# melspectrum007/audio-visual-speech-enhancement

Measured on AMD Instinct MI355X. Metric: clips/sec (STFT+CNN forward) on 200-ms@16kHz segments, 1/2/4/8 MI355X, higher is better.
Workload: dtype fp32_split

## Files before the change

audio-visual-speech-enhancement_amd/csrc/avse_common.h:

```cpp
#pragma once
#include <hip/hip_runtime.h>
#include <stdint.h>
#include <string>

typedef __bf16 bf16_t;
typedef __bf16 bf16x8 __attribute__((ext_vector_type(8)));
typedef _Float16 f16x8 __attribute__((ext_vector_type(8)));
typedef _Float16 f16x4 __attribute__((ext_vector_type(4)));
typedef float f32x4 __attribute__((ext_vector_type(4)));
typedef int i32x4 __attribute__((ext_vector_type(4)));

struct avse_ctx;

namespace avse {

void set_error(const std::string& msg);

int ctx_device_index(const struct ::avse_ctx* c);

int ensure_lds_attr(const void* fn, int bytes);

struct Options {
    int no_gemm = 0;
    int no_audenc = 0;
    int no_dechead = 0;
    int no_dectail = 0;
    int unfused_tail = 0;
    int no_halo = 0;
    int mfma32 = 0;
    int serial = 0;
    int graph = 0;
    int gemm_ksplit_cap = 0;
    int dense_istft = 0;
    int no_act_scale = 0;
    int no_win = 0;
    int no_v1p = 0;
    int no_a1valu = 0;
    int side_prio = 0;
};

#define AVSE_HIP_CHECK(expr)                                                                   \
    do {                                                                                       \
        hipError_t _e = (expr);                                                                \
        if (_e != hipSuccess) {                                                                \
            ::avse::set_error(std::string(#expr " failed: ") + hipGetErrorString(_e));         \
            return 2;                                                        \
        }                                                                                      \
    } while (0)

struct DebugHit {
    unsigned hit, kernel, code, block, thread;
    int value, expect;
};
enum DebugKernel : unsigned {
    DK_V1R = 1,
    DK_SPEC = 3,
    DK_ISTFT = 4,
};
#ifdef AVSE_DEBUG
inline constexpr bool kDebugBuild = true;
__device__ __forceinline__ void debug_record(DebugHit* h, unsigned kern, unsigned code, int value, int expect) {
    if (atomicCAS(&h->hit, 0u, 1u) == 0u) {
        h->kernel = kern;
        h->code = code;
        h->block = blockIdx.x;
        h->thread = threadIdx.x;
        h->value = value;
        h->expect = expect;
        __threadfence();
    }
}
#define AVSE_DEBUG_RECORD(reader)                                                                    \
    static __device__ ::avse::DebugHit g_avse_dbg;                                                   \
    int reader(::avse::DebugHit* out) {                                                              \
        ::avse::DebugHit zero{};                                                                     \
        if (hipMemcpyFromSymbol(out, HIP_SYMBOL(g_avse_dbg), sizeof(zero)) != hipSuccess) return 2;   \
        return hipMemcpyToSymbol(HIP_SYMBOL(g_avse_dbg), &zero, sizeof(zero)) == hipSuccess ? 0 : 2; \
    }
#define AVSE_CHECK_DEV(cond, kern, code, value, expect)                                              \
    do {                                                                                             \
        if (!(cond)) ::avse::debug_record(&g_avse_dbg, (kern), (code), (int)(value), (int)(expect)); \
    } while (0)
#else
inline constexpr bool kDebugBuild = false;
#define AVSE_DEBUG_RECORD(reader)              \
    int reader(::avse::DebugHit* out) {          \
        *out = ::avse::DebugHit{};               \
        return 0;                                \
    }
#define AVSE_CHECK_DEV(cond, kern, code, value, expect) \
// ... 168 lines not shown
    const bf16_t* w1;
    const bf16_t* w2;
    const bf16_t* w3;
    const float* sc[3];
    const float* sh[3];
};
bool dec_head_supported(const DecHeadArgs& a);
int launch_dec_head(const DecHeadArgs& a, hipStream_t s);

struct GemmArgs {
    const bf16_t* a;
    long long lda;
    const bf16_t* w;
    int M, N, kpad;
    const float* scale;
    const float* shift;
    int act;
    bf16_t* out;
    long long ldo;
    int out_off;
    int ksplit;
    float* partial;
    int* counters;
    int split;
    int slabs_per_split;
    unsigned* range_flag;
    unsigned range_bit;
};
int gemm_ksplit(int M, int N, int kpad, int cap);
int gemm_s16_ksplit(int N, int kpad, int* slabs_per_split);
size_t gemm_ws_bytes(int M, int N, int kpad, int cap);
int launch_gemm(const GemmArgs& g, int mode, hipStream_t s);
int launch_aud_enc(const AudEncArgs& a, hipStream_t s);
int launch_dec_tail(const DecTailArgs& a, hipStream_t s);

enum HaloVariant { HALO_NONE = -1, HALO_V1 = 0, HALO_K5 = 1, HALO_K3_16 = 2, HALO_K3_8 = 3, HALO_V1P = 4 };
enum HaloOut { OUT_BF16 = 0, OUT_S16 = 1, OUT_F32 = 2 };

struct HaloArgs {
    int variant;
    const void* in;
    const float* video;
    const float* vmean;
    const float* vstd;
    void* out;
    const void* w;
    const float* scale;
    const float* shift;
    int N, Hc, Wc, Ci, Co;
    long long out_clip_stride;
    int out_pix_stride;
    int out_c_off;
    int mfma32;
    int split;
    int out_mode;
    unsigned long long* prof;
    unsigned* range_flag;
    unsigned range_bit, range_in_bit;
};

int launch_conv_stream(const HaloArgs& a, hipStream_t s);
int launch_conv_v1r(const HaloArgs& a, hipStream_t s);
int launch_video_prep(const float* video, const float* mean, const float* stdv, void* out, int64_t N,
                      int F, int dtype, hipStream_t s);
int launch_audio_prep(const float* audio, void* out, int64_t npix, int dtype, hipStream_t s);
int launch_aconv1_split(const float* in, const float* w, const float* scale, const float* shift, void* out, int64_t N,
                        int H, int W, int Ho, int Wo, int KH, int KW, int S, int pt, int pl, int Co, unsigned* range_flag,
                        unsigned range_bit, unsigned range_in_bit, hipStream_t s);
int launch_out_conv(const void* in, const float* w64, float bias, float* out, int64_t npix, int dtype,
                    hipStream_t s);
int launch_broadcast_row(const void* src, void* dst, int64_t rows, int64_t row_bytes, int64_t stride_bytes,
                         hipStream_t s);
int launch_video_normalize(float* video, int64_t S, int H, int W, int F, const float* mean,
                           const float* stdv, hipStream_t s);
int launch_mse(const float* a, const float* b, int64_t n, float* loss, float* partial, hipStream_t s);

size_t mix_pairs_scratch_bytes(int64_t n_pairs);
int launch_mix_pairs(const int16_t* speech, const int64_t* speech_off, const int16_t* noise, const int64_t* noise_off,
                     const double* snr_lin, int64_t n_pairs, int64_t L, float* rows, double* mix64, double* factor,
                     void* scratch, hipStream_t s);
constexpr int kVideoStatsMaxF = 8;
size_t video_stats_scratch_bytes(int64_t S, int H, int W);
int launch_video_stats(const float* video, int64_t S, int H, int W, int F, float* mean, float* stdv, void* scratch,
                       hipStream_t s);

}
```

audio-visual-speech-enhancement_amd/csrc/capi.hip:

```cpp
#include <algorithm>
#include <atomic>
#include <cmath>
#include <cstdio>
#include <cstdlib>
#include <cstring>
#include <mutex>
#include <set>
#include <string>
#include <utility>
#include <vector>

#include "../../include/avse.h"
#include "avse_common.h"
#include "netplan.h"

namespace avse {
static thread_local std::string g_err;
void set_error(const std::string& msg) { g_err = msg; }

int ensure_lds_attr(const void* fn, int bytes) {
    static std::mutex mu;
    static std::set<std::pair<const void*, int>> done;
    int dev = 0;
    AVSE_HIP_CHECK(hipGetDevice(&dev));
// ... 112 lines not shown
    struct Graph {
        const void* key[9];
        int64_t n;
        Options opt;
        hipGraphExec_t exec;
    };
    std::vector<Graph> graphs;
    hipStream_t cap = nullptr;
};

namespace avse {
int ctx_device_index(const avse_ctx* c) { return c->device; }
}

struct GpuLayer {
    LayerDef def;
    int cin_pad = 0;
    int hq = 0, wq = 0, ho = 0, wo = 0;
    int nphase = 1;
    ConvPhase ph[MAX_PHASES];
    void* w = nullptr;
    float* scale = nullptr;
    float* shift = nullptr;
    int2* taps = nullptr;
    int halo = HALO_NONE;
    void* w_halo = nullptr;
    void* w_dense = nullptr;
    float* w_f32 = nullptr;
    float* scale_h = nullptr;
    int2 htaps[MAX_TAPS * MAX_PHASES] = {};
};

struct OptionName {
    const char* name;
    const char* env;
    int Options::*field;
};
const OptionName kOptionNames[] = {
    {"no_gemm", "AVSE_NO_GEMM", &Options::no_gemm},
    {"no_audenc", "AVSE_NO_AUDENC", &Options::no_audenc},
    {"no_dechead", "AVSE_NO_DECHEAD", &Options::no_dechead},
    {"no_dectail", "AVSE_NO_DECTAIL", &Options::no_dectail},
    {"unfused_tail", "AVSE_UNFUSED_TAIL", &Options::unfused_tail},
    {"no_halo", "AVSE_NO_HALO", &Options::no_halo},
    {"mfma32", "AVSE_MFMA32", &Options::mfma32},
    {"serial", "AVSE_SERIAL", &Options::serial},
    {"graph", "AVSE_GRAPH", &Options::graph},
    {"gemm_ksplit_cap", "AVSE_GEMM_KSPLIT", &Options::gemm_ksplit_cap},
    {"dense_istft", "AVSE_DENSE_ISTFT", &Options::dense_istft},
    {"no_act_scale", "AVSE_NO_ACT_SCALE", &Options::no_act_scale},
    {"no_win", "AVSE_NO_WIN", &Options::no_win},
    {"no_v1p", "AVSE_NO_V1P", &Options::no_v1p},
    {"no_a1valu", "AVSE_NO_A1VALU", &Options::no_a1valu},
    {"side_prio", "AVSE_SIDE_PRIO", &Options::side_prio},
};

struct avse_weights {
    int dtype = 0;
    int device = 0;
    uint64_t serial = 0;
    NetPlan plan = kPlan25;
    GpuLayer layers[kNumLayers - 1];
    float* d6_w = nullptr;
    float d6_bias = 0.f;
    mutable std::atomic<void*> vzero_emb{nullptr};
    mutable std::mutex vzero_mu;
    mutable unsigned vzero_range = 0;
    int act_exp[kNumLayers] = {};
    std::vector<float> blob;
    mutable avse_weights* f32_twin = nullptr;
    mutable std::mutex twin_mu;
    std::vector<void*> allocs;
    ~avse_weights();
};

avse_weights::~avse_weights() {
    delete f32_twin;
    (void)hipFree(vzero_emb.load());
    for (void* p : allocs) (void)hipFree(p);
}

namespace {

template <typename T>
int upload(avse_weights* W, const std::vector<T>& h, T** out) {
    void* p = nullptr;
    if (hipMalloc(&p, sizeof(T) * (h.empty() ? 1 : h.size())) != hipSuccess) return fail(AVSE_ERR_OOM, "hipMalloc failed (weights)");
    W->allocs.push_back(p);
    if (!h.empty() && hipMemcpy(p, h.data(), sizeof(T) * h.size(), hipMemcpyHostToDevice) != hipSuccess)
        return fail(AVSE_ERR_HIP, "hipMemcpy failed (weights)");
    *out = (T*)p;
    return 0;
}

struct Arena {
    size_t off[32];
    size_t per_clip_bytes;
};
enum Buf { B_VIN, B_AIN, B_A1, B_A2, B_A3, B_A4, B_V1, B_V2, B_V3, B_V4, B_V5, B_CAT, B_E1, B_E2, B_E3,
           B_D1, B_D2, B_D3, B_D4, B_D5, B_COUNT };
size_t buf_elems(const NetPlan& p, int b) {
    const size_t T = p.T, w1 = (T + 1) / 2, w3 = p.W5;
    const size_t e[B_COUNT] = {128 * 128 * 8, 80 * T * 8, 40 * w1 * 64, 40 * w1 * 64, 20 * w3 * 128,
                               10 * w3 * 128, 64 * 64 * 128, 32 * 32 * 128, 16 * 16 * 256, 8 * 8 * 256,
                               4 * 4 * 512, (size_t)p.cat, (size_t)p.emb, (size_t)p.emb, (size_t)p.aemb,
                               10 * w3 * 128, 20 * w3 * 128, 40 * 2 * w3 * 128, 40 * 2 * w3 * 64, 80 * 4 * w3 * 64};
// ... 532 lines not shown
                            const uint16_t h = f2h(v);
                            sp[((size_t)st * L.cout + n) * 32 + kk] = h;
                            sp[((size_t)st * L.cout + n) * 32 + 16 + kk] = f2h(v - h2f(h));
                        }
            }
            if ((rc = upload(W, scale_h, &G.scale_h))) return rc;
            uint16_t* d;
            if ((rc = upload(W, sp, &d))) return rc;
            G.w_halo = d;
            return 0;
        }
        if ((rc = upload(W, scale_h, &G.scale_h))) return rc;
        std::vector<uint16_t> hp;
        if (G.halo == HALO_V1) {
            hp.assign((size_t)L.kh * L.cout * 32, 0);
            for (int ky = 0; ky < L.kh; ++ky)
                for (int n = 0; n < L.cout; ++n)
                    for (int kx = 0; kx < L.kw; ++kx)
                        for (int f = 0; f < L.cin; ++f)
                            hp[((size_t)ky * L.cout + n) * 32 + kx * 6 + f] =
                                f2bf(sgn[n] * kernel[((size_t)(ky * L.kw + kx) * L.cin + f) * L.cout + n]);
        } else {
            const int nsteps = (L.cin / 128) * 4 * ntap;
            hp.assign((size_t)nsteps * L.cout * 32, 0);
            for (int st = 0; st < nsteps; ++st)
                for (int n = 0; n < L.cout; ++n)
                    for (int kk = 0; kk < 32; ++kk) {
                        const int tap = st % ntap, chunk = st / ntap;
                        const int c = chunk * 32 + kk;
                        hp[((size_t)st * L.cout + n) * 32 + kk] =
                            f2bf(sgn[n] * kernel[((size_t)tap * L.cin + c) * L.cout + n]);
                    }
        }
        uint16_t* d;
        if ((rc = upload(W, hp, &d))) return rc;
        G.w_halo = d;
    }
    return 0;
}

HaloArgs halo_args(const GpuLayer& G, const void* in, const float* video, const float* vmean, const float* vstd,
                   void* out, long long out_clip_stride, int out_pix_stride, int out_c_off, int64_t N,
                   const Options& opt) {
    HaloArgs a;
    std::memset(&a, 0, sizeof(a));
    a.variant = G.halo;
    a.in = in;
    a.video = video;
    a.vmean = vmean;
    a.vstd = vstd;
    a.out = out;
    a.w = G.w_halo;
    a.mfma32 = opt.mfma32;
    a.scale = G.scale_h;
    a.shift = G.shift;
    a.N = (int)N;
    a.Hc = G.def.hin;
    a.Wc = G.def.win;
    a.Ci = G.def.cin;
    a.Co = G.def.cout;
    a.out_clip_stride = out_clip_stride;
    a.out_pix_stride = out_pix_stride;
    a.out_c_off = out_c_off;
    return a;
}

DecTailArgs dec_tail_args(const GpuLayer& G4, const GpuLayer& G5, const avse_weights* W, const void* in, float* out,
                          int64_t N) {
    DecTailArgs a;
    std::memset(&a, 0, sizeof(a));
    a.in = reinterpret_cast<const bf16_t*>(in);
    a.out = out;
    a.N = (int)N;
    auto extents = [](const GpuLayer& G, int p, int& dy0, int& dy1, int& dx0, int& dx1) {
        dy0 = dx0 = 1 << 20;
        dy1 = dx1 = -(1 << 20);
        for (int t = 0; t < G.ph[p].ntaps; ++t) {
            const int2 d = G.htaps[G.ph[p].tap_off + t];
            dy0 = std::min(dy0, d.x); dy1 = std::max(dy1, d.x);
            dx0 = std::min(dx0, d.y); dx1 = std::max(dx1, d.y);
        }
    };
    a.w4 = reinterpret_cast<const bf16_t*>(G4.w);
    a.sc4 = G4.scale;
    a.sh4 = G4.shift;
    a.nt4 = G4.ph[0].ntaps;
    a.kpad4 = G4.ph[0].kpad;
    int dy0, dy1, dx0, dx1;
    extents(G4, 0, dy0, dy1, dx0, dx1);
    a.pt4 = -dy0; a.pl4 = -dx0; a.rows4 = G4.hq + dy1 - dy0; a.pitch4 = G4.wq + dx1 - dx0;
    bool grid_ok = true;
    auto tap_grid = [&](const GpuLayer& G, int p, int& dy, int& dx, int& nx) {
        const int2* t = G.htaps + G.ph[p].tap_off;
        const int nt = G.ph[p].ntaps;
        dy = t[0].x;
        dx = t[0].y;
        nx = 1;
        while (nx < nt && t[nx].x == dy) ++nx;
        for (int k = 0; k < nt; ++k)
            if (t[k].x != dy - k / nx || t[k].y != dx - k % nx) grid_ok = false;
    };
    tap_grid(G4, 0, a.dy4, a.dx4, a.nx4);
    a.w5 = reinterpret_cast<const bf16_t*>(G5.w);
    a.sc5 = G5.scale;
    a.sh5 = G5.shift;
    int ey0 = 1 << 20, ey1 = -(1 << 20), ex0 = 1 << 20, ex1 = -(1 << 20);
// ... 899 lines not shown
```

audio-visual-speech-enhancement_amd/csrc/conv_stream.hip:

```cpp
#include <cstdlib>
#include <type_traits>

#include "avse_common.h"

namespace avse {
namespace {

constexpr float LRELU = 0.3f;
constexpr int kOOB = 0x7fffff00;

typedef float f32x16 __attribute__((ext_vector_type(16)));

template <bool M16> __device__ __forceinline__ int wswz(int row) { return M16 ? 2 * ((row >> 2) & 1) : (row >> 2) & 3; }
template <bool M16> __device__ __forceinline__ int hsw(int y) { return M16 ? 2 * (y & 1) : y & 3; }

__device__ __forceinline__ __amdgpu_buffer_rsrc_t make_rsrc(const void* base, long long bytes) {
    const int nrec = bytes > kOOB ? kOOB : (bytes < 0 ? 0 : (int)bytes);
    return __builtin_amdgcn_make_buffer_rsrc(const_cast<void*>(base), (short)0, nrec, 0x00020000);
}

#ifndef AVSE_HALO_AUX
#define AVSE_HALO_AUX 0
#endif
#ifndef AVSE_WGT_AUX
#define AVSE_WGT_AUX 0
#endif
__device__ __forceinline__ i32x4 ld16(__amdgpu_buffer_rsrc_t rs, int voff, int soff) {
    return __builtin_amdgcn_raw_buffer_load_b128(rs, voff, soff, AVSE_HALO_AUX);
}
__device__ __forceinline__ i32x4 ld16w(__amdgpu_buffer_rsrc_t rs, int voff, int soff) {
    return __builtin_amdgcn_raw_buffer_load_b128(rs, voff, soff, AVSE_WGT_AUX);
}
__device__ __forceinline__ void st16(char* p, i32x4 v) { *reinterpret_cast<i32x4*>(p) = v; }

template <int N>
__device__ __forceinline__ void wait_vm_lgkm0() {
    static_assert(N >= 0 && N < 64, "vmcnt range");
    asm volatile("s_waitcnt vmcnt(%0) lgkmcnt(0)" ::"n"(N) : "memory");
}
__device__ __forceinline__ void barrier_raw() { asm volatile("s_barrier" ::: "memory"); }

template <int KS, int TH, int TW, int NCLIP, int LAT_ = (KS == 5 ? 10 : 6), int BP_ = 1, bool S16_ = false>
struct StreamGeom {
    static constexpr int HH = TH + KS - 1, HW = TW + KS - 1;
    static constexpr int HPIX = NCLIP * HH * HW;
    static constexpr int HPIECES = (HPIX * 64 + 1023) / 1024;
    static constexpr int HPW = (HPIECES + 3) / 4;
    static constexpr int NTAP = KS * KS;
    static constexpr int CSLOT = HPIECES * 1024;
    static constexpr int WSLOT = 8192;
    static constexpr int LAT = LAT_, BP = BP_, NWS = S16_ ? 2 * BP + 1 : 2 * BP, WD = LAT + BP + 1, NHS = 3,
                         PAIR = ((2 * NTAP) % BP ? 4 : 2) * NTAP, CPI = PAIR / NTAP;
    static_assert(PAIR % BP == 0, "barrier periods align with the unrolled loader iteration");
    static_assert(BP == 1 || BP == 2 || (S16_ && BP == 4), "barrier period");
    static_assert(!S16_ || BP % 2 == 0, "split-f16 operands: whole slice pairs per barrier");
    static constexpr int LDS = NHS * CSLOT + NWS * WSLOT;
    static_assert(LDS + 1024 <= 160 * 1024, "LDS");
    static_assert(NCLIP * TH * TW == 256, "tile = 256 conv pixels (4 waves x 4 fragments)");
    static_assert(PAIR % LAT == 0 && LAT < NTAP, "the ring set of a step is compile-time");
    static_assert(HPW <= NTAP && HPW - 1 + LAT + BP - 1 <= 2 * NTAP - (S16_ ? BP + 1 : 2), "halo pieces must land in time");
    static constexpr int loads(int j, int abl) {
        const int tap = ((j % NTAP) + NTAP) % NTAP;
        return ((abl & 2) ? 0 : 2) + ((!(abl & 1) && tap < HPW) ? 1 : 0);
    }
    static constexpr int vm_wait(int j, int abl) {
        int n = 0;
        for (int i = j - LAT + 2; i <= j; ++i) n += loads(i, abl);
        return n;
    }
};

template <int KS, int TH, int TW, int NCLIP, bool M16 = true, int LAT_ = StreamGeom<KS, TH, TW, NCLIP>::LAT, int ABL = 0,
          int BP_ = 1, bool S16 = false>
__global__ __launch_bounds__(512, 1) void k_conv_stream(HaloArgs a) {
    static_assert(!S16 || M16, "split-f16 operands: 16x16x32 compute waves only");
    using G = StreamGeom<KS, TH, TW, NCLIP, LAT_, BP_, S16>;
    constexpr int HH = G::HH, HW = G::HW, HPIX = G::HPIX, HPW = G::HPW, NTAP = G::NTAP;
    constexpr int CSLOT = G::CSLOT, WSLOT = G::WSLOT, LAT = G::LAT, WD = G::WD, PAIR = G::PAIR;
    constexpr int BP = G::BP, NWS = G::NWS;
    constexpr int BPR = TW / 8, BPC = (TH / 4) * BPR;
    static_assert(TW % 8 == 0 && TH % 4 == 0 && BPC % 2 == 0, "a wave's two blocks share their y origin mod 4");
    constexpr int PAD = (KS - 1) / 2;

    extern __shared__ __attribute__((aligned(1024))) char lds[];
    char* const halo = lds;
    char* const wring = lds + G::NHS * CSLOT;

    const int tid = threadIdx.x;
    const int lane = tid & 63;
    const int wave = __builtin_amdgcn_readfirstlane(tid >> 6);
    const int w = wave & 3;

    const int nch = a.Ci / 32;
    const int spt = nch * NTAP;
    const int tiles_x = a.Wc / TW, tiles_y = a.Hc / TH;
    const int tiles_per_clip = tiles_x * tiles_y;
    const int ntiles = ((a.N + NCLIP - 1) / NCLIP) * tiles_per_clip;
    const int gxs = (int)gridDim.x;
    const int slot = (gxs % 8 == 0) ? ((int)blockIdx.x % 8) * (gxs / 8) + (int)blockIdx.x / 8 : (int)blockIdx.x;
    const int nmine = (ntiles - slot + gxs - 1) / gxs;
    if (nmine <= 0) return;
    const int nchunks = nmine * nch;
    const int co0 = blockIdx.y * 128;
    const long long clip_bytes = (long long)a.Hc * a.Wc * a.Ci * 2;

    auto tile_origin = [&](int k, int& clip0, int& oy0, int& ox0) {
        const int t = slot + k * gxs;
        clip0 = (ABL & 64) ? 0 : (t / tiles_per_clip) * NCLIP;
        const int tt = t % tiles_per_clip;
        oy0 = (tt / tiles_x) * TH;
        ox0 = (tt % tiles_x) * TW;
    };

    if (wave >= 4) {
        const __amdgpu_buffer_rsrc_t wrs = make_rsrc(reinterpret_cast<const char*>(a.w) + (size_t)co0 * 64,
                                                     (long long)spt * a.Co * 64 - (long long)co0 * 64);
        const int wslice = a.Co * 64, wend = spt * wslice;
        int wvoff[2];
#pragma unroll
        for (int u = 0; u < 2; ++u) {
            const int row = 32 * w + 16 * u + (lane >> 2), sl = lane & 3;
            wvoff[u] = row * 64 + ((sl ^ wswz<M16>(row)) << 4);
        }
        char* const wdst = wring + 2048 * w + lane * 16;
        auto tile_rsrc = [&](int clip0) {
            return make_rsrc(reinterpret_cast<const char*>(a.in) + (long long)clip0 * clip_bytes,
                             (long long)(a.N - clip0) * clip_bytes);
        };
        const int ci2 = a.Ci * 2, hc = a.Hc, wc = a.Wc;
        auto tile_voffs = [&](int oy0, int ox0, int (&vo)[HPW]) {
#pragma unroll
            for (int pc = 0; pc < HPW; ++pc) {
                const int P = w + 4 * pc;
                const int p = P * 16 + (lane >> 2), sl = lane & 3;
                const int cl = p / (HH * HW), rr = p - cl * (HH * HW);
                const int y = rr / HW, x = rr - y * HW;
                const int iy = oy0 + y - PAD, ix = ox0 + x - PAD;
                const int off = ((cl * hc + iy) * wc + ix) * ci2 + ((sl ^ hsw<M16>(y)) << 4);
                const bool ok = (P < G::HPIECES) & (p < HPIX) & ((unsigned)iy < (unsigned)hc) & ((unsigned)ix < (unsigned)wc);
                vo[pc] = ok ? off : kOOB;
            }
        };
        auto piece_store = [&](auto pcc, char* base, i32x4 v) {
            constexpr int pc = decltype(pcc)::value;
            if constexpr (4 * pc + 3 < G::HPIECES) st16(base + pc * 4096, v);
            else if (w + 4 * pc < G::HPIECES) st16(base + pc * 4096, v);
        };

        int cur_clip0, cur_oy0, cur_ox0, nxt_clip0, nxt_oy0, nxt_ox0;
        tile_origin(0, cur_clip0, cur_oy0, cur_ox0);
        tile_origin(1, nxt_clip0, nxt_oy0, nxt_ox0);
        __amdgpu_buffer_rsrc_t cur_rs = tile_rsrc(cur_clip0), nxt_rs = tile_rsrc(nxt_clip0);
        int vo_cur[HPW], vo_nxt[HPW];
        tile_voffs(cur_oy0, cur_ox0, vo_cur);
        tile_voffs(nxt_oy0, nxt_ox0, vo_nxt);
        char* const pbase0 = halo + w * 1024 + lane * 16;

        [&]<int... PC>(std::integer_sequence<int, PC...>) {
            (piece_store(std::integral_constant<int, PC>{}, pbase0, ld16(cur_rs, vo_cur[PC], 0)), ...);
            ((PC < NTAP - LAT ? piece_store(std::integral_constant<int, PC>{}, pbase0 + CSLOT, ld16(cur_rs, vo_cur[PC], 64))
                              : (void)0), ...);
        }(std::make_integer_sequence<int, HPW>{});
#pragma unroll
        for (int s = 0; s <= BP; ++s)
#pragma unroll
            for (int u = 0; u < 2; ++u) st16(wdst + s * WSLOT + 1024 * u, ld16w(wrs, wvoff[u], (s % spt) * wslice));
        i32x4 rw[LAT][2], rp[LAT];
        [&]<int... S>(std::integer_sequence<int, S...>) {
            ([&] {
                 rw[S][0] = ld16w(wrs, wvoff[0], ((S + BP + 1) % spt) * wslice);
                 rw[S][1] = ld16w(wrs, wvoff[1], ((S + BP + 1) % spt) * wslice);
                 constexpr int vt = NTAP - LAT + S;
                 if constexpr (vt < HPW && !(ABL & 1)) rp[S] = ld16(cur_rs, vo_cur[vt < HPW ? vt : 0], 64);
             }(), ...);
        }(std::make_integer_sequence<int, LAT>{});
        wait_vm_lgkm0<0>();
        barrier_raw();
        barrier_raw();

        int k = 0, c = 0, g = 0, hs2 = 2;
        int woff = (WD % spt) * wslice;
        constexpr bool kRot = PAIR % NWS != 0;
        int wrot = 0;
        int vsel[HPW];
        __amdgpu_buffer_rsrc_t prs = cur_rs;
        int psoff = 0;
        char* pd_cur = pbase0 + CSLOT;
        char* pd_prev = pd_cur;
        unsigned long long ptp = (ABL & 128) ? __builtin_amdgcn_s_memtime() : 0, pt0 = 0, pt1 = 0, p_work = 0,
                           p_wait = 0, p_bar = 0;
        auto chunk_begin = [&]() {
            const bool nx = c + 2 >= nch;
            const bool real = g + 2 < nchunks;
#pragma unroll
            for (int pc = 0; pc < HPW; ++pc) vsel[pc] = !real ? kOOB : nx ? vo_nxt[pc] : vo_cur[pc];
            prs = nx ? nxt_rs : cur_rs;
            psoff = (nx ? c + 2 - nch : c + 2) * 64;
            pd_prev = pd_cur;
            pd_cur = pbase0 + hs2 * CSLOT;
        };
        auto chunk_end = [&]() {
            ++g;
            hs2 = hs2 == 2 ? 0 : hs2 + 1;
            if (++c == nch) {
                c = 0;
                ++k;
                cur_oy0 = nxt_oy0;
                cur_ox0 = nxt_ox0;
                cur_rs = nxt_rs;
#pragma unroll
                for (int pc = 0; pc < HPW; ++pc) vo_cur[pc] = vo_nxt[pc];
                tile_origin(k + 1, nxt_clip0, nxt_oy0, nxt_ox0);
                nxt_rs = tile_rsrc(nxt_clip0);
                tile_voffs(nxt_oy0, nxt_ox0, vo_nxt);
            }
        };
        auto lstep = [&](auto jidx) {
            constexpr int j = decltype(jidx)::value;
            constexpr int tap = j % NTAP, S = j % LAT;
            constexpr int jl = j - LAT;
            constexpr int tl = ((jl % NTAP) + NTAP) % NTAP;
            constexpr bool lprev = (jl < 0) || (jl / NTAP != j / NTAP);
            if constexpr (tap == 0) chunk_begin();
            if constexpr (!(ABL & 2)) {
                int wsl = (j + BP + 1) % NWS + (kRot ? wrot : 0);
                if (wsl >= NWS) wsl -= NWS;
                char* const wd = wdst + wsl * WSLOT;
                st16(wd, rw[S][0]);
                st16(wd + 1024, rw[S][1]);
            }
            if constexpr (tl < HPW && !(ABL & 1))
                piece_store(std::integral_constant<int, (tl < HPW ? tl : 0)>{}, lprev ? pd_prev : pd_cur, rp[S]);
            if constexpr (!(ABL & 2)) {
                rw[S][0] = ld16w(wrs, wvoff[0], woff);
                rw[S][1] = ld16w(wrs, wvoff[1], woff);
            }
            if constexpr (tap < HPW && !(ABL & 1)) rp[S] = ld16(prs, vsel[tap < HPW ? tap : 0], psoff);
            woff += wslice;
            if (woff == wend) woff = 0;
            if constexpr (!(ABL & 4) && j % BP == BP - 1) {
                if constexpr ((ABL & 128) != 0) pt0 = __builtin_amdgcn_s_memtime();
                wait_vm_lgkm0<G::vm_wait(j, ABL)>();
                if constexpr ((ABL & 128) != 0) pt1 = __builtin_amdgcn_s_memtime();
                barrier_raw();
                if constexpr ((ABL & 128) != 0) {
                    const unsigned long long pt2 = __builtin_amdgcn_s_memtime();
                    p_work += pt0 - ptp;
                    p_wait += pt1 - pt0;
                    p_bar += pt2 - pt1;
                    ptp = pt2;
                }
            }
            if constexpr (tap == NTAP - 1) chunk_end();
        };
        for (int pr = 0; pr < nchunks; pr += G::CPI) {
            [&]<int... J>(std::integer_sequence<int, J...>) {
                (lstep(std::integral_constant<int, J>{}), ...);
            }(std::make_integer_sequence<int, PAIR>{});
            if constexpr (kRot) wrot = (wrot + PAIR) % NWS;
        }
        wait_vm_lgkm0<0>();
        if constexpr ((ABL & 128) != 0)
            if (lane == 0) {
                unsigned long long* pr = a.prof + ((size_t)blockIdx.x * 8 + wave) * 4;
                pr[0] = p_work; pr[1] = p_wait; pr[2] = p_bar; pr[3] = (unsigned long long)nchunks * NTAP;
            }
        return;
    }

    __builtin_amdgcn_s_setprio(2);
    if constexpr (M16) {
        constexpr int SBX = TW / 4, SB = (TH / 4) * SBX;
        static_assert(TH % 4 == 0 && TW % 4 == 0 && (SBX % 4 == 0 || SBX == 2) && SB % 4 == 0, "block geometry");
        const int r16 = lane & 15, kg = lane >> 4;
        const int q = r16 >> 2, dy = (r16 >> 1) & 1, dx = r16 & 1;
        const int b0 = 4 * w, cl0 = b0 / SB, bb0 = b0 % SB;
        const int by0 = bb0 / SBX, bx0 = bb0 % SBX;
        const int ab = ((cl0 * HH + 4 * by0 + 2 * (q >> 1) + dy) * HW + 4 * bx0 + 2 * (q & 1) + dx) * 64;
// ... 30 lines not shown
#pragma unroll
        for (int i = 0; i < 4; ++i)
#pragma unroll
            for (int j = 0; j < 8; ++j) acc[i][j] = (f32x4){};
        const int Wp = a.Wc / 2;
        bool range_bad = false;
        auto epilogue_m = [&](auto modec, int clip0, int oy0, int ox0) {
            constexpr int OM = decltype(modec)::value;
            constexpr int ES = OM == OUT_F32 ? 4 : 2;
            const long long cbytes = a.out_clip_stride * ES;
            const __amdgpu_buffer_rsrc_t ors = make_rsrc(reinterpret_cast<const char*>(a.out) + (long long)clip0 * cbytes,
                                                         (long long)(a.N - clip0) * cbytes);
            const int cbase = cl0 * (int)a.out_clip_stride + a.out_c_off + (OM == OUT_S16 ? 2 * co0 : co0) + r16;
#pragma unroll
            for (int i = 0; i < 4; ++i) {
                const int py = (oy0 + 4 * (by0 + i / SBX)) / 2 + (kg >> 1);
                const int px = (ox0 + 4 * (bx0 + i % SBX)) / 2 + (kg & 1);
                const int pbase = cbase + (py * Wp + px) * a.out_pix_stride;
#pragma unroll
                for (int j = 0; j < 8; ++j) {
                    const float mx = fmaxf(fmaxf(acc[i][j][0], acc[i][j][1]), fmaxf(acc[i][j][2], acc[i][j][3]));
                    float x = fmaf(mx, ssh[16 * j + r16], ssh[128 + 16 * j + r16]);
                    x = fmaxf(x, LRELU * x);
                    if constexpr (OM == OUT_BF16) {
                        __builtin_amdgcn_raw_buffer_store_b16(__builtin_bit_cast(unsigned short, (bf16_t)x), ors,
                                                              (pbase + 16 * j) * 2, 0, 0);
                    } else if constexpr (OM == OUT_S16) {
                        const _Float16 h = (_Float16)x;
                        const _Float16 l = (_Float16)(x - (float)h);
                        range_bad |= pair_out_of_range(x);
                        __builtin_amdgcn_raw_buffer_store_b16(__builtin_bit_cast(unsigned short, h), ors,
                                                              (pbase + 32 * j) * 2, 0, 0);
                        __builtin_amdgcn_raw_buffer_store_b16(__builtin_bit_cast(unsigned short, l), ors,
                                                              (pbase + 32 * j + 16) * 2, 0, 0);
                    } else {
                        __builtin_amdgcn_raw_buffer_store_b32(__builtin_bit_cast(int, x), ors, (pbase + 16 * j) * 4, 0, 0);
                    }
                    acc[i][j] *= 0.f;
                }
            }
        };
        auto epilogue = [&](int clip0, int oy0, int ox0) {
            if constexpr (!S16) {
                epilogue_m(std::integral_constant<int, OUT_BF16>{}, clip0, oy0, ox0);
            } else if (a.out_mode == OUT_S16) {
                epilogue_m(std::integral_constant<int, OUT_S16>{}, clip0, oy0, ox0);
            } else {
                epilogue_m(std::integral_constant<int, OUT_F32>{}, clip0, oy0, ox0);
            }
        };

        unsigned long long ptp = (ABL & 128) ? __builtin_amdgcn_s_memtime() : 0, pt0 = 0, pt1 = 0, p_work = 0,
                           p_wait = 0, p_bar = 0;
        int tap1 = 1, hs1 = 0;
        i32x4 fa[4], fb[8], na[4], nb[8];
        frags(0, 0, 0, fa, fb);
        if constexpr ((ABL & 8) != 0) frags(0, 0, 0, na, nb);
        asm volatile("s_waitcnt lgkmcnt(0)" ::: "memory");
        barrier_raw();

        auto cstep = [&](auto bar, int t, i32x4 (&ca)[4], i32x4 (&cb)[8], i32x4 (&xa)[4], i32x4 (&xb)[8]) {
            if constexpr (!S16) {
                if constexpr (!(ABL & 8)) frags(hs1, tap1, (t + 1) & (NWS - 1), xa, xb);
                if constexpr (!(ABL & 16))
#pragma unroll
                    for (int i = 0; i < 4; ++i)
#pragma unroll
                        for (int j = 0; j < 8; ++j)
                            acc[i][j] = __builtin_amdgcn_mfma_f32_16x16x32_bf16(
                                __builtin_bit_cast(bf16x8, ca[i]), __builtin_bit_cast(bf16x8, cb[j]), acc[i][j], 0, 0, 0);
            }
            if constexpr (!S16) {
#pragma unroll
                for (int r = 0; r < 12; ++r) {
                    __builtin_amdgcn_sched_group_barrier(0x008, 1, 0);
                    __builtin_amdgcn_sched_group_barrier(0x100, 1, 0);
                }
                __builtin_amdgcn_sched_group_barrier(0x008, 20, 0);
                __builtin_amdgcn_sched_barrier(0);
            }
            if constexpr (!(ABL & 4) && decltype(bar)::value) {
                if constexpr ((ABL & 128) != 0) pt0 = __builtin_amdgcn_s_memtime();
                asm volatile("s_waitcnt lgkmcnt(0)" ::: "memory");
                if constexpr ((ABL & 128) != 0) pt1 = __builtin_amdgcn_s_memtime();
                barrier_raw();
                if constexpr ((ABL & 128) != 0) {
                    const unsigned long long pt2 = __builtin_amdgcn_s_memtime();
                    p_work += pt0 - ptp;
                    p_wait += pt1 - pt0;
                    p_bar += pt2 - pt1;
                    ptp = pt2;
                }
            }
            if (++tap1 == NTAP) {
                tap1 = 0;
                hs1 = hs1 == 2 ? 0 : hs1 + 1;
            }
        };
        int t = 0;
        int cur_clip0, cur_oy0, cur_ox0;
        if constexpr (S16) {
            auto advance = [&]() {
                if (++tap1 == NTAP) {
                    tap1 = 0;
                    hs1 = hs1 == 2 ? 0 : hs1 + 1;
                }
            };
            auto mfma_group = [&](const i32x4 (&ca)[4], const i32x4 (&cb)[8]) {
                if constexpr (!(ABL & 16))
#pragma unroll
                    for (int j = 0; j < 8; ++j)
#pragma unroll
                        for (int i = 0; i < 4; ++i)
                            acc[i][j] = __builtin_amdgcn_mfma_f32_16x16x32_f16(
                                __builtin_bit_cast(f16x8, ca[i]), __builtin_bit_cast(f16x8, cb[j]), acc[i][j], 0, 0, 0);
            };
            auto sched = [](auto nds, auto per) {
                constexpr int ND = decltype(nds)::value, PER = decltype(per)::value;
#pragma unroll
                for (int r = 0; r < ND; ++r) {
                    __builtin_amdgcn_sched_group_barrier(0x008, PER, 0);
                    __builtin_amdgcn_sched_group_barrier(0x100, 1, 0);
                }
                __builtin_amdgcn_sched_group_barrier(0x008, 32 - ND * PER, 0);
                __builtin_amdgcn_sched_barrier(0);
            };
            const bool hi_half = kg >= 2;
            auto pstep = [&](auto bar, int t, i32x4 (&a0)[4], i32x4 (&b0)[8], i32x4 (&na)[4], i32x4 (&nb)[8]) {
                i32x4 a1[4], b1[8], bp[8];
                const int ws0 = t % NWS, ws1 = (t + 1) % NWS, ws2 = (t + 2) % NWS;
                if constexpr (!(ABL & 8)) frags(hs1, tap1, ws1, a1, b1);
                advance();
                mfma_group(a0, b0);
                sched(std::integral_constant<int, 12>{}, std::integral_constant<int, 1>{});
                if constexpr (!(ABL & 8)) frags_lo(hi_half ? ws1 : ws0, bp);
                mfma_group(a1, b1);
                sched(std::integral_constant<int, 8>{}, std::integral_constant<int, 2>{});
#pragma unroll
                for (int i = 0; i < 4; ++i)
#pragma unroll
                    for (int d = 0; d < 4; ++d)
                        a0[i][d] = (int)__builtin_amdgcn_permlane32_swap((unsigned)a0[i][d], (unsigned)a1[i][d], false,
                                                                         false)[0];
                if constexpr (!(ABL & 8)) frags(hs1, tap1, ws2, na, nb);
                advance();
                mfma_group(a0, bp);
                sched(std::integral_constant<int, 12>{}, std::integral_constant<int, 1>{});
                if constexpr (!(ABL & 4) && decltype(bar)::value) {
                    if constexpr ((ABL & 128) != 0) pt0 = __builtin_amdgcn_s_memtime();
                    asm volatile("s_waitcnt lgkmcnt(0)" ::: "memory");
                    if constexpr ((ABL & 128) != 0) pt1 = __builtin_amdgcn_s_memtime();
                    barrier_raw();
                    if constexpr ((ABL & 128) != 0) {
                        const unsigned long long pt2 = __builtin_amdgcn_s_memtime();
                        p_work += pt0 - ptp;
                        p_wait += pt1 - pt0;
                        p_bar += pt2 - pt1;
                        ptp = pt2;
                    }
                }
            };
            for (int kt = 0; kt < nmine; ++kt) {
                for (int s = 0; s < spt; s += 4, t += 4) {
                    pstep(std::bool_constant<BP == 2>{}, t, fa, fb, na, nb);
                    pstep(std::true_type{}, t + 2, na, nb, fa, fb);
                }
                tile_origin(kt, cur_clip0, cur_oy0, cur_ox0);
                epilogue(cur_clip0, cur_oy0, cur_ox0);
            }
        } else {
            for (int kt = 0; kt < nmine; ++kt) {
                for (int s = 0; s < spt; s += 2, t += 2) {
                    cstep(std::bool_constant<BP == 1>{}, t, fa, fb, na, nb);
                    cstep(std::true_type{}, t + 1, na, nb, fa, fb);
                }
                tile_origin(kt, cur_clip0, cur_oy0, cur_ox0);
                epilogue(cur_clip0, cur_oy0, cur_ox0);
            }
        }
        if constexpr ((ABL & 128) != 0)
            if (lane == 0) {
                unsigned long long* pr = a.prof + ((size_t)blockIdx.x * 8 + wave) * 4;
                pr[0] = p_work; pr[1] = p_wait; pr[2] = p_bar; pr[3] = (unsigned long long)t;
            }
        if constexpr (S16) range_report(a.range_flag, a.range_bit, range_bad);
        return;
    }
    const int r32 = lane & 31, hi = lane >> 5;
    int ab;
    {
        const int b = 2 * w;
        const int cl = b / BPC, bb = b % BPC;
        const int q = r32 >> 2;
        const int y = 4 * (bb / BPR) + 2 * (q >> 2) + ((r32 >> 1) & 1);
        const int x = 8 * (bb % BPR) + 2 * (q & 3) + (r32 & 1);
        ab = ((cl * HH + y) * HW + x) * 64;
    }
    constexpr int blk1 = ((4 * (1 / BPR)) * HW + 8 * (1 % BPR)) * 64;
    const int ylo = 2 * ((r32 >> 4) & 1) + ((r32 >> 1) & 1);
    int boffm[2];
#pragma unroll
    for (int m = 0; m < 2; ++m) boffm[m] = r32 * 64 + (((2 * m + hi) ^ wswz<M16>(r32)) << 4);
    auto frags = [&](int hs, int tap, int ws, i32x4 (&fa)[4], i32x4 (&fb)[8]) {
        const int ky = tap / KS, kx = tap % KS;
        const int sw = hsw<M16>(ylo + ky);
        const char* hp = halo + hs * CSLOT + ab + (ky * HW + kx) * 64;
        const char* wp = wring + ws * WSLOT;
#pragma unroll
        for (int m = 0; m < 2; ++m) {
            const int pos = ((2 * m + hi) ^ sw) << 4;
#pragma unroll
            for (int i = 0; i < 2; ++i) fa[2 * i + m] = *reinterpret_cast<const i32x4*>(hp + i * blk1 + pos);
#pragma unroll
            for (int jb = 0; jb < 4; ++jb) fb[2 * jb + m] = *reinterpret_cast<const i32x4*>(wp + boffm[m] + 2048 * jb);
        }
    };
    float sc[4], sh[4];
#pragma unroll
// ... 59 lines not shown
            __builtin_amdgcn_sched_group_barrier(0x008, 1, 0);
            __builtin_amdgcn_sched_group_barrier(0x100, 1, 0);
        }
        __builtin_amdgcn_sched_group_barrier(0x008, 4, 0);
        __builtin_amdgcn_sched_barrier(0);
        if constexpr (!(ABL & 4) && decltype(bar)::value) {
            if constexpr ((ABL & 128) != 0) pt0 = __builtin_amdgcn_s_memtime();
            asm volatile("s_waitcnt lgkmcnt(0)" ::: "memory");
            if constexpr ((ABL & 128) != 0) pt1 = __builtin_amdgcn_s_memtime();
            barrier_raw();
            if constexpr ((ABL & 128) != 0) {
                const unsigned long long pt2 = __builtin_amdgcn_s_memtime();
                p_work += pt0 - ptp;
                p_wait += pt1 - pt0;
                p_bar += pt2 - pt1;
                ptp = pt2;
            }
        }
        if (++tap1 == NTAP) {
            tap1 = 0;
            hs1 = hs1 == 2 ? 0 : hs1 + 1;
        }
    };
    int t = 0;
    int cur_clip0, cur_oy0, cur_ox0;
    using BAR0 = std::bool_constant<BP == 1>;
    for (int kt = 0; kt < nmine; ++kt) {
        cstep(std::true_type{}, BAR0{}, t, fa, fb, na, nb);
        cstep(std::false_type{}, std::true_type{}, t + 1, na, nb, fa, fb);
        t += 2;
        for (int s = 2; s < spt; s += 2, t += 2) {
            cstep(std::false_type{}, BAR0{}, t, fa, fb, na, nb);
            cstep(std::false_type{}, std::true_type{}, t + 1, na, nb, fa, fb);
        }
        tile_origin(kt, cur_clip0, cur_oy0, cur_ox0);
        epilogue(cur_clip0, cur_oy0, cur_ox0);
    }
    if constexpr ((ABL & 128) != 0)
        if (lane == 0) {
            unsigned long long* pr = a.prof + ((size_t)blockIdx.x * 8 + wave) * 4;
            pr[0] = p_work; pr[1] = p_wait; pr[2] = p_bar; pr[3] = (unsigned long long)t;
        }
}

#ifndef AVSE_S16_BP5
#define AVSE_S16_BP5 4
#endif
#ifndef AVSE_S16_BP3
#define AVSE_S16_BP3 4
#endif
#ifndef AVSE_S16_LAT3
#define AVSE_S16_LAT3 4
#endif
template <int KS, int TH, int TW, int NCLIP, bool M16, bool S16 = false>
int launch_stream(const HaloArgs& a, hipStream_t s) {
    constexpr int BP = S16 ? (KS == 5 ? AVSE_S16_BP5 : AVSE_S16_BP3) : 1;
    constexpr int LAT = (S16 && KS == 3) ? AVSE_S16_LAT3 : StreamGeom<KS, TH, TW, NCLIP>::LAT;
    using G = StreamGeom<KS, TH, TW, NCLIP, LAT, BP, S16>;
    constexpr auto kern = k_conv_stream<KS, TH, TW, NCLIP, M16, G::LAT, 0, BP, S16>;
    if (int rc = ensure_lds_attr((const void*)kern, G::LDS + 1024)) return rc;
    if (a.Hc % TH || a.Wc % TW || a.Co % 128 || a.Ci % 64) {
        set_error("stream conv: tile does not divide the layer");
        return 3;
    }
    int dev = 0, ncu = 256;
    (void)hipGetDevice(&dev);
    (void)hipDeviceGetAttribute(&ncu, hipDeviceAttributeMultiprocessorCount, dev);
    const int tiles = ((a.N + NCLIP - 1) / NCLIP) * (a.Hc / TH) * (a.Wc / TW);
    const int cob = a.Co / 128;
    int gx = ncu / cob;
    gx = gx >= 8 ? gx / 8 * 8 : (gx < 1 ? 1 : gx);
    if (gx > tiles) gx = tiles;
    if ((a.Ci / 32) % G::CPI || (S16 && ((a.out_mode != OUT_S16 && a.out_mode != OUT_F32) || (a.Ci / 32 * KS * KS) % 4))) {
        set_error("stream conv: split-f16 operands write split or f32 outputs, over slice counts divisible by 4");
        return 3;
    }
    hipLaunchKernelGGL(kern, dim3(gx, cob), dim3(512), G::LDS + 1024, s, a);
    AVSE_HIP_CHECK(hipGetLastError());
    return 0;
}

}

int launch_conv_stream(const HaloArgs& a, hipStream_t s) {
    const bool m32 = a.mfma32 != 0;
    if (a.split) {
        switch (a.variant) {
            case HALO_K5: return launch_stream<5, 16, 16, 1, true, true>(a, s);
            case HALO_K3_16: return launch_stream<3, 16, 16, 1, true, true>(a, s);
            case HALO_K3_8: return launch_stream<3, 8, 8, 4, true, true>(a, s);
        }
        set_error("stream conv: unsupported variant");
        return 3;
    }
    switch (a.variant) {
        case HALO_K5: return m32 ? launch_stream<5, 16, 16, 1, false>(a, s) : launch_stream<5, 16, 16, 1, true>(a, s);
        case HALO_K3_16: return m32 ? launch_stream<3, 16, 16, 1, false>(a, s) : launch_stream<3, 16, 16, 1, true>(a, s);
        case HALO_K3_8: return m32 ? launch_stream<3, 8, 8, 4, false>(a, s) : launch_stream<3, 8, 8, 4, true>(a, s);
    }
    set_error("stream conv: unsupported variant");
    return 3;
}

}
```

Baseline: 79330.

## Add planar slice-pair pipeline for split-f16 streaming conv kernels

Adds a planar variant of the split-f16 streaming convolution main loop. It computes LDS fragment offsets incrementally with XOR-based half selection and interleaves the hi/lo fragment reads with the MFMA groups, instead of recomputing frags per step. The weight ring gains one extra look-ahead slot, with a new compile-time check that halo pieces land in time. The variant is on by default for split layers and can be disabled with AVSE_NO_PLANAR. It aims to cut address arithmetic and LDS read latency in the inner loop, at the cost of more LDS ring slots and more complex scheduling.

Result: faster. 81160, median of 6 (+2.3%).

```diff
diff --git a/audio-visual-speech-enhancement_amd/csrc/avse_common.h b/audio-visual-speech-enhancement_amd/csrc/avse_common.h
--- a/audio-visual-speech-enhancement_amd/csrc/avse_common.h
+++ b/audio-visual-speech-enhancement_amd/csrc/avse_common.h
@@ -36,6 +36,7 @@
     int no_win = 0;
     int no_v1p = 0;
     int no_a1valu = 0;
+    int no_planar = 0;
     int side_prio = 0;
 };
 
@@ -310,6 +311,7 @@
     int out_pix_stride;
     int out_c_off;
     int mfma32;
+    int no_planar;
     int split;
     int out_mode;
     unsigned long long* prof;
diff --git a/audio-visual-speech-enhancement_amd/csrc/capi.hip b/audio-visual-speech-enhancement_amd/csrc/capi.hip
--- a/audio-visual-speech-enhancement_amd/csrc/capi.hip
+++ b/audio-visual-speech-enhancement_amd/csrc/capi.hip
@@ -188,6 +188,7 @@
     {"no_win", "AVSE_NO_WIN", &Options::no_win},
     {"no_v1p", "AVSE_NO_V1P", &Options::no_v1p},
     {"no_a1valu", "AVSE_NO_A1VALU", &Options::no_a1valu},
+    {"no_planar", "AVSE_NO_PLANAR", &Options::no_planar},
     {"side_prio", "AVSE_SIDE_PRIO", &Options::side_prio},
 };
 
@@ -826,6 +827,7 @@
     a.out = out;
     a.w = G.w_halo;
     a.mfma32 = opt.mfma32;
+    a.no_planar = opt.no_planar;
     a.scale = G.scale_h;
     a.shift = G.shift;
     a.N = (int)N;
diff --git a/audio-visual-speech-enhancement_amd/csrc/conv_stream.hip b/audio-visual-speech-enhancement_amd/csrc/conv_stream.hip
--- a/audio-visual-speech-enhancement_amd/csrc/conv_stream.hip
+++ b/audio-visual-speech-enhancement_amd/csrc/conv_stream.hip
@@ -40,7 +40,7 @@
 }
 __device__ __forceinline__ void barrier_raw() { asm volatile("s_barrier" ::: "memory"); }
 
-template <int KS, int TH, int TW, int NCLIP, int LAT_ = (KS == 5 ? 10 : 6), int BP_ = 1, bool S16_ = false>
+template <int KS, int TH, int TW, int NCLIP, int LAT_ = (KS == 5 ? 10 : 6), int BP_ = 1, bool S16_ = false, bool PL_ = false>
 struct StreamGeom {
     static constexpr int HH = TH + KS - 1, HW = TW + KS - 1;
     static constexpr int HPIX = NCLIP * HH * HW;
@@ -49,8 +49,9 @@
     static constexpr int NTAP = KS * KS;
     static constexpr int CSLOT = HPIECES * 1024;
     static constexpr int WSLOT = 8192;
-    static constexpr int LAT = LAT_, BP = BP_, NWS = S16_ ? 2 * BP + 1 : 2 * BP, WD = LAT + BP + 1, NHS = 3,
-                         PAIR = ((2 * NTAP) % BP ? 4 : 2) * NTAP, CPI = PAIR / NTAP;
+    static_assert(!PL_ || S16_, "planar slice pairs: split-f16 operands only");
+    static constexpr int LAT = LAT_, BP = BP_, WAH = BP + (PL_ ? 2 : 1), NWS = PL_ ? 2 * BP + 2 : S16_ ? 2 * BP + 1 : 2 * BP,
+                         WD = LAT + WAH, NHS = 3, PAIR = ((2 * NTAP) % BP ? 4 : 2) * NTAP, CPI = PAIR / NTAP;
     static_assert(PAIR % BP == 0, "barrier periods align with the unrolled loader iteration");
     static_assert(BP == 1 || BP == 2 || (S16_ && BP == 4), "barrier period");
     static_assert(!S16_ || BP % 2 == 0, "split-f16 operands: whole slice pairs per barrier");
@@ -58,7 +59,16 @@
     static_assert(LDS + 1024 <= 160 * 1024, "LDS");
     static_assert(NCLIP * TH * TW == 256, "tile = 256 conv pixels (4 waves x 4 fragments)");
     static_assert(PAIR % LAT == 0 && LAT < NTAP, "the ring set of a step is compile-time");
-    static_assert(HPW <= NTAP && HPW - 1 + LAT + BP - 1 <= 2 * NTAP - (S16_ ? BP + 1 : 2), "halo pieces must land in time");
+    static constexpr bool planar_halo_in_time() {
+        for (int g = 0; g < 2 * BP; ++g) {
+            const int s0 = g * NTAP, visible = ((s0 + HPW - 1 + LAT) / BP + 1) * BP;
+            const int first_read = (((s0 + 2 * NTAP) & ~1) - 2) / BP * BP;
+            if (visible > first_read) return false;
+        }
+        return LAT >= BP;
+    }
+    static_assert(HPW <= NTAP && (PL_ ? planar_halo_in_time() : HPW - 1 + LAT + BP - 1 <= 2 * NTAP - (S16_ ? BP + 1 : 2)),
+                  "halo pieces must land in time");
     static constexpr int loads(int j, int abl) {
         const int tap = ((j % NTAP) + NTAP) % NTAP;
         return ((abl & 2) ? 0 : 2) + ((!(abl & 1) && tap < HPW) ? 1 : 0);
@@ -71,10 +81,10 @@
 };
 
 template <int KS, int TH, int TW, int NCLIP, bool M16 = true, int LAT_ = StreamGeom<KS, TH, TW, NCLIP>::LAT, int ABL = 0,
-          int BP_ = 1, bool S16 = false>
+          int BP_ = 1, bool S16 = false, int PL = 0>
 __global__ __launch_bounds__(512, 1) void k_conv_stream(HaloArgs a) {
     static_assert(!S16 || M16, "split-f16 operands: 16x16x32 compute waves only");
-    using G = StreamGeom<KS, TH, TW, NCLIP, LAT_, BP_, S16>;
+    using G = StreamGeom<KS, TH, TW, NCLIP, LAT_, BP_, S16, PL != 0>;
     constexpr int HH = G::HH, HW = G::HW, HPIX = G::HPIX, HPW = G::HPW, NTAP = G::NTAP;
     constexpr int CSLOT = G::CSLOT, WSLOT = G::WSLOT, LAT = G::LAT, WD = G::WD, PAIR = G::PAIR;
     constexpr int BP = G::BP, NWS = G::NWS;
@@ -162,14 +172,14 @@
                               : (void)0), ...);
         }(std::make_integer_sequence<int, HPW>{});
 #pragma unroll
-        for (int s = 0; s <= BP; ++s)
+        for (int s = 0; s < G::WAH; ++s)
 #pragma unroll
             for (int u = 0; u < 2; ++u) st16(wdst + s * WSLOT + 1024 * u, ld16w(wrs, wvoff[u], (s % spt) * wslice));
         i32x4 rw[LAT][2], rp[LAT];
         [&]<int... S>(std::integer_sequence<int, S...>) {
             ([&] {
-                 rw[S][0] = ld16w(wrs, wvoff[0], ((S + BP + 1) % spt) * wslice);
-                 rw[S][1] = ld16w(wrs, wvoff[1], ((S + BP + 1) % spt) * wslice);
+                 rw[S][0] = ld16w(wrs, wvoff[0], ((S + G::WAH) % spt) * wslice);
+                 rw[S][1] = ld16w(wrs, wvoff[1], ((S + G::WAH) % spt) * wslice);
                  constexpr int vt = NTAP - LAT + S;
                  if constexpr (vt < HPW && !(ABL & 1)) rp[S] = ld16(cur_rs, vo_cur[vt < HPW ? vt : 0], 64);
              }(), ...);
@@ -223,7 +233,7 @@
             constexpr bool lprev = (jl < 0) || (jl / NTAP != j / NTAP);
             if constexpr (tap == 0) chunk_begin();
             if constexpr (!(ABL & 2)) {
-                int wsl = (j + BP + 1) % NWS + (kRot ? wrot : 0);
+                int wsl = (j + G::WAH) % NWS + (kRot ? wrot : 0);
                 if (wsl >= NWS) wsl -= NWS;
                 char* const wd = wdst + wsl * WSLOT;
                 st16(wd, rw[S][0]);
@@ -360,10 +370,56 @@
 
         unsigned long long ptp = (ABL & 128) ? __builtin_amdgcn_s_memtime() : 0, pt0 = 0, pt1 = 0, p_work = 0,
                            p_wait = 0, p_bar = 0;
-        int tap1 = 1, hs1 = 0;
+        int tap1 = PL ? 0 : 1, hs1 = 0;
         i32x4 fa[4], fb[8], na[4], nb[8];
-        frags(0, 0, 0, fa, fb);
-        if constexpr ((ABL & 8) != 0) frags(0, 0, 0, na, nb);
+        const bool hi_half = kg >= 2;
+        const int ac0 = ab + (((kg & 1) ^ hsw<true>(dy)) << 4);
+        const int bc0 = G::NHS * CSLOT + (hi_half ? WSLOT : 0) + bo16;
+        static_assert(PL == 0 || (CSLOT % 64 == 0 && WSLOT % 64 == 0 && NWS % 2 == 0), "the xor forms of the l-half offsets");
+        int abase = ac0, bbase = bc0, us0 = 0, us1 = 0, ps0 = 0, ps1 = 0, wsc = 0;
+        auto advance = [&]() {
+            if (++tap1 == NTAP) {
+                tap1 = 0;
+                hs1 = hs1 == 2 ? 0 : hs1 + 1;
+            }
+        };
+        auto next_pair = [&]() {
+            const int ky0 = tap1 / KS, kx0 = tap1 % KS;
+            const int u0 = hs1 * CSLOT + (ky0 * HW + kx0) * 64;
+            ps0 = (ky0 & 1) << 5;
+            advance();
+            const int ky1 = tap1 / KS, kx1 = tap1 % KS;
+            const int u1 = hs1 * CSLOT + (ky1 * HW + kx1) * 64;
+            ps1 = (ky1 & 1) << 5;
+            advance();
+            abase += hi_half ? u1 - us1 : u0 - us0;
+            us0 = u0;
+            us1 = u1;
+        };
+        auto aoff_h = [&]() { return abase ^ (hi_half ? ps1 : ps0); };
+        auto rd_a = [&](int off, i32x4 (&f)[4]) {
+            const char* hp = halo + off;
+#pragma unroll
+            for (int i = 0; i < 4; ++i) f[i] = *reinterpret_cast<const i32x4*>(hp + boff_of(i));
+        };
+        auto rd_b = [&](int off, i32x4 (&f)[8]) {
+            const char* wp = lds + off;
+#pragma unroll
+            for (int j = 0; j < 8; ++j)
+                f[j] = ((ABL & 256) && j >= 4) ? f[j - 4] : *reinterpret_cast<const i32x4*>(wp + 1024 * j);
+        };
+        if constexpr (PL != 0) {
+            next_pair();
+            rd_a(aoff_h(), fa);
+            rd_b(bbase, fb);
+            if constexpr ((ABL & 8) != 0) {
+                rd_a(aoff_h() ^ 32, na);
+                rd_b(bbase ^ 32, nb);
+            }
+        } else {
+            frags(0, 0, 0, fa, fb);
+            if constexpr ((ABL & 8) != 0) frags(0, 0, 0, na, nb);
+        }
         asm volatile("s_waitcnt lgkmcnt(0)" ::: "memory");
         barrier_raw();
 
@@ -408,12 +464,6 @@
         int t = 0;
         int cur_clip0, cur_oy0, cur_ox0;
         if constexpr (S16) {
-            auto advance = [&]() {
-                if (++tap1 == NTAP) {
-                    tap1 = 0;
-                    hs1 = hs1 == 2 ? 0 : hs1 + 1;
-                }
-            };
             auto mfma_group = [&](const i32x4 (&ca)[4], const i32x4 (&cb)[8]) {
                 if constexpr (!(ABL & 16))
 #pragma unroll
@@ -433,7 +483,6 @@
                 __builtin_amdgcn_sched_group_barrier(0x008, 32 - ND * PER, 0);
                 __builtin_amdgcn_sched_barrier(0);
             };
-            const bool hi_half = kg >= 2;
             auto pstep = [&](auto bar, int t, i32x4 (&a0)[4], i32x4 (&b0)[8], i32x4 (&na)[4], i32x4 (&nb)[8]) {
                 i32x4 a1[4], b1[8], bp[8];
                 const int ws0 = t % NWS, ws1 = (t + 1) % NWS, ws2 = (t + 2) % NWS;
@@ -468,10 +517,45 @@
                     }
                 }
             };
+            auto ppl = [&](auto bar, i32x4 (&ah)[4], i32x4 (&al)[4], i32x4 (&bh)[8], i32x4 (&bl)[8]) {
+                if constexpr (!(ABL & 8)) rd_a(aoff_h() ^ 32, al);
+                mfma_group(ah, bh);
+                sched(std::integral_constant<int, 4>{}, std::integral_constant<int, 1>{});
+                if constexpr (!(ABL & 8)) rd_b(bbase ^ 32, bl);
+                mfma_group(al, bh);
+                sched(std::integral_constant<int, 8>{}, std::integral_constant<int, 1>{});
+                bbase += wsc + 2 == NWS ? -(NWS - 2) * WSLOT : 2 * WSLOT;
+                wsc = wsc + 2 == NWS ? 0 : wsc + 2;
+                next_pair();
+                if constexpr (!(ABL & 8)) {
+                    rd_a(aoff_h(), al);
+                    rd_b(bbase, bh);
+                }
+                mfma_group(ah, bl);
+                sched(std::integral_constant<int, 12>{}, std::integral_constant<int, 1>{});
+                if constexpr (!(ABL & 4) && decltype(bar)::value) {
+                    if constexpr ((ABL & 128) != 0) pt0 = __builtin_amdgcn_s_memtime();
+                    asm volatile("s_waitcnt lgkmcnt(0)" ::: "memory");
+                    if constexpr ((ABL & 128) != 0) pt1 = __builtin_amdgcn_s_memtime();
+                    barrier_raw();
+                    if constexpr ((ABL & 128) != 0) {
+                        const unsigned long long pt2 = __builtin_amdgcn_s_memtime();
+                        p_work += pt0 - ptp;
+                        p_wait += pt1 - pt0;
+                        p_bar += pt2 - pt1;
+                        ptp = pt2;
+                    }
+                }
+            };
             for (int kt = 0; kt < nmine; ++kt) {
                 for (int s = 0; s < spt; s += 4, t += 4) {
-                    pstep(std::bool_constant<BP == 2>{}, t, fa, fb, na, nb);
-                    pstep(std::true_type{}, t + 2, na, nb, fa, fb);
+                    if constexpr (PL != 0) {
+                        ppl(std::bool_constant<BP == 2>{}, fa, na, fb, nb);
+                        ppl(std::true_type{}, na, fa, fb, nb);
+                    } else {
+                        pstep(std::bool_constant<BP == 2>{}, t, fa, fb, na, nb);
+                        pstep(std::true_type{}, t + 2, na, nb, fa, fb);
+                    }
                 }
                 tile_origin(kt, cur_clip0, cur_oy0, cur_ox0);
                 epilogue(cur_clip0, cur_oy0, cur_ox0);
@@ -637,12 +721,12 @@
 #ifndef AVSE_S16_LAT3
 #define AVSE_S16_LAT3 4
 #endif
-template <int KS, int TH, int TW, int NCLIP, bool M16, bool S16 = false>
+template <int KS, int TH, int TW, int NCLIP, bool M16, bool S16 = false, int PL = 0>
 int launch_stream(const HaloArgs& a, hipStream_t s) {
     constexpr int BP = S16 ? (KS == 5 ? AVSE_S16_BP5 : AVSE_S16_BP3) : 1;
     constexpr int LAT = (S16 && KS == 3) ? AVSE_S16_LAT3 : StreamGeom<KS, TH, TW, NCLIP>::LAT;
-    using G = StreamGeom<KS, TH, TW, NCLIP, LAT, BP, S16>;
-    constexpr auto kern = k_conv_stream<KS, TH, TW, NCLIP, M16, G::LAT, 0, BP, S16>;
+    using G = StreamGeom<KS, TH, TW, NCLIP, LAT, BP, S16, PL != 0>;
+    constexpr auto kern = k_conv_stream<KS, TH, TW, NCLIP, M16, G::LAT, 0, BP, S16, PL>;
     if (int rc = ensure_lds_attr((const void*)kern, G::LDS + 1024)) return rc;
     if (a.Hc % TH || a.Wc % TW || a.Co % 128 || a.Ci % 64) {
         set_error("stream conv: tile does not divide the layer");
@@ -670,10 +754,11 @@
 int launch_conv_stream(const HaloArgs& a, hipStream_t s) {
     const bool m32 = a.mfma32 != 0;
     if (a.split) {
+        const bool pl = a.no_planar == 0;
         switch (a.variant) {
-            case HALO_K5: return launch_stream<5, 16, 16, 1, true, true>(a, s);
-            case HALO_K3_16: return launch_stream<3, 16, 16, 1, true, true>(a, s);
-            case HALO_K3_8: return launch_stream<3, 8, 8, 4, true, true>(a, s);
+            case HALO_K5: return pl ? launch_stream<5, 16, 16, 1, true, true, 1>(a, s) : launch_stream<5, 16, 16, 1, true, true>(a, s);
+            case HALO_K3_16: return pl ? launch_stream<3, 16, 16, 1, true, true, 1>(a, s) : launch_stream<3, 16, 16, 1, true, true>(a, s);
+            case HALO_K3_8: return pl ? launch_stream<3, 8, 8, 4, true, true, 1>(a, s) : launch_stream<3, 8, 8, 4, true, true>(a, s);
         }
         set_error("stream conv: unsupported variant");
         return 3;
```
